# Z-Zheng/ever

Measured on AMD Instinct MI355X. Metric: 512x512 tiles/sec fwd+bwd, FarSeg-R50, higher is better.
Workload: dtype f32; 1 GPU; FarSeg ResNet-50 FPN (FarSegHead defaults, BCE+dice), 3-band 512x512, batch 16/GPU, fwd+bwd+SGD step, inputs resident in HBM; global_batch=16, parallelism=single

## Files before the change

ever_amd/csrc/bn.hip:

```cpp
#include "bn_common.hpp"

namespace evk {

__global__ __launch_bounds__(256) void bn_stats_partial_kernel(const float* __restrict__ x, float* __restrict__ partial,
                                                               int64_t rows, int C, int64_t rows_per_blk, int tpc,
                                                               int rl) {
  __shared__ f32x4 red[2][256];
  const int c4 = C >> 2;
  const int tc = threadIdx.x % tpc, tr = threadIdx.x / tpc;
  const int64_t r0 = (int64_t)blockIdx.x * rows_per_blk;
  const int64_t r1 = min(rows, r0 + rows_per_blk);
  for (int cb = tc; cb < c4; cb += tpc) {
    f32x4 s = {0.f, 0.f, 0.f, 0.f}, q = {0.f, 0.f, 0.f, 0.f};
    const f32x4 pv = *reinterpret_cast<const f32x4*>(x + cb * 4);
    if (tr < rl) {
      int64_t r = r0 + tr;
      const int64_t st = rl;
      for (; r + 3 * st < r1; r += 4 * st) {
        const f32x4 v0 = *reinterpret_cast<const f32x4*>(x + r * C + cb * 4) - pv;
        const f32x4 v1 = *reinterpret_cast<const f32x4*>(x + (r + st) * C + cb * 4) - pv;
        const f32x4 v2 = *reinterpret_cast<const f32x4*>(x + (r + 2 * st) * C + cb * 4) - pv;
        const f32x4 v3 = *reinterpret_cast<const f32x4*>(x + (r + 3 * st) * C + cb * 4) - pv;
        s += (v0 + v1) + (v2 + v3);
        q += (v0 * v0 + v1 * v1) + (v2 * v2 + v3 * v3);
// ... 159 lines not shown
        const f32x4 x0 = bp_ld(x + o0), x1 = bp_ld(x + o1);
        const f32x4 x2 = bp_ld(x + o2), x3 = bp_ld(x + o3);
        f32x4 y0 = zero4, y1 = zero4, y2 = zero4, y3 = zero4;
        if (relu == 1) {
          y0 = bp_ld(y + o0);
          y1 = bp_ld(y + o1);
          y2 = bp_ld(y + o2);
          y3 = bp_ld(y + o3);
        }
        one(g0, x0, y0, o0);
        one(g1, x1, y1, o1);
        one(g2, x2, y2, o2);
        one(g3, x3, y3, o3);
      }
      for (; r < r1; r += st) {
        const size_t o0 = (size_t)r * C + cb * 4;
        const f32x4 g0 = bp_ld(dy + o0);
        const f32x4 x0 = bp_ld(x + o0);
        const f32x4 y0 = (relu == 1) ? bp_ld(y + o0) : zero4;
        one(g0, x0, y0, o0);
      }
    }
    fold_store_record(red, s, q, partial, bn_blk(), C, cb, tc, tr, tpc, rl);
    if constexpr (PK) {
      red[0][threadIdx.x] = gm;
      red[1][threadIdx.x] = xm;
      __syncthreads();
      if (tr == 0) {
        for (int k = 1; k < rl; ++k) {
          const f32x4 a = red[0][k * tpc + tc], b = red[1][k * tpc + tc];
          gm.x = fmaxf(gm.x, a.x); gm.y = fmaxf(gm.y, a.y); gm.z = fmaxf(gm.z, a.z); gm.w = fmaxf(gm.w, a.w);
          xm.x = fmaxf(xm.x, b.x); xm.y = fmaxf(xm.y, b.y); xm.z = fmaxf(xm.z, b.z); xm.w = fmaxf(xm.w, b.w);
        }
        float* o = pmax + (size_t)bn_blk() * 2 * C;
        *reinterpret_cast<f32x4*>(o + cb * 4) = gm;
        *reinterpret_cast<f32x4*>(o + C + cb * 4) = xm;
      }
      __syncthreads();
    }
  }
}

template <int FC = kFinCh>
__global__ __launch_bounds__(256) void bn_bwd_final_kernel(const float* __restrict__ partial, int nblk, int C,
                                                           double inv_rows, const float* __restrict__ gamma,
                                                           const float* __restrict__ invstd,
                                                           float* __restrict__ dgamma, float* __restrict__ dbeta,
                                                           float* __restrict__ coef, int train,
                                                           uint32_t* __restrict__ amax,
                                                           const float* __restrict__ pmax) {
  if (!pmax) zero_amax(amax);
  float gmax = 0.f, xmax = 0.f;
  if (pmax) {
    __shared__ float mred[4][FC];
    const int tc = threadIdx.x % FC, tl = threadIdx.x / FC;
    const int cc = bn_fin_group() * FC + tc;
    if (cc < C) {
      const float* pm = pmax + cc;
      const size_t st = (size_t)2 * C;
      int b = tl;
      for (; b + 3 * (256 / FC) < nblk; b += 4 * (256 / FC)) {
        const float g0 = pm[b * st], g1 = pm[(b + (256 / FC)) * st], g2 = pm[(b + 2 * (256 / FC)) * st],
                    g3 = pm[(b + 3 * (256 / FC)) * st];
        const float x0 = pm[b * st + C], x1 = pm[(b + (256 / FC)) * st + C], x2 = pm[(b + 2 * (256 / FC)) * st + C],
                    x3 = pm[(b + 3 * (256 / FC)) * st + C];
        gmax = fmaxf(gmax, fmaxf(fmaxf(g0, g1), fmaxf(g2, g3)));
        xmax = fmaxf(xmax, fmaxf(fmaxf(x0, x1), fmaxf(x2, x3)));
      }
      for (; b < nblk; b += (256 / FC)) {
        gmax = fmaxf(gmax, pm[b * st]);
        xmax = fmaxf(xmax, pm[b * st + C]);
      }
    }
    auto mx = [](float a, float b) { return fmaxf(a, b); };
    gmax = fold_channel_lanes<FC>(gmax, mred, mx);
    xmax = fold_channel_lanes<FC>(xmax, mred, mx);
  }
  int c;
  double s, q;
  if (!reduce_partials<FC>(partial, nblk, C, c, s, q)) return;
  if (dbeta) dbeta[c] = (float)s;
  if (dgamma) dgamma[c] = (float)q;
  const float g = gamma ? gamma[c] : 1.f;
  const float k0 = g * invstd[c], k1 = train ? (float)(s * inv_rows) : 0.f, k2 = train ? (float)(q * inv_rows) : 0.f;
  coef[c] = k0;
  coef[C + c] = k1;
  coef[2 * C + c] = k2;
  if (pmax) {
    const float bound = fabsf(k0) * (gmax + fabsf(k1) + xmax * fabsf(k2));
    uint32_t bits = __builtin_bit_cast(uint32_t, bound);
    if (bound != bound) bits = 0x7fc00000u;
    if (bits) atomicMax(&amax[0], bits);
  }
}

template <bool PK>
__global__ __launch_bounds__(256) void bn_bwd_apply_kernel(const float* __restrict__ dy, const float* __restrict__ x,
                                                           const float* __restrict__ y, const float* __restrict__ mean,
                                                           const float* __restrict__ invstd,
                                                           const float* __restrict__ coef,
                                                           const float* __restrict__ gamma,
                                                           const float* __restrict__ beta, float* __restrict__ dx,
                                                           size_t n4, int C, int relu, uint32_t* __restrict__ amax,
                                                           const uint32_t* __restrict__ bits = nullptr) {
  const size_t base = (size_t)bn_blk() * 256;
  const size_t i = base + threadIdx.x;
  const bool valid = i < n4;
  f32x4 out = {0.f, 0.f, 0.f, 0.f};
  float pk_inv = 1.f;
  if constexpr (PK) pk_inv = op_scale(amax[0]).inv;
  if (valid) {
    const int c4 = C >> 2;
    const int c = chunk_of(base, c4);
// ... 94 lines not shown
  const double unbias = rows > 1.0 ? rows / (rows - 1.0) : 1.0;
  if (running_mean) running_mean[c] = (1.f - momentum) * running_mean[c] + momentum * meanf;
  if (running_var) running_var[c] = (1.f - momentum) * running_var[c] + momentum * (float)(var * unbias);
  const float g = gamma ? gamma[c] : 1.f, bb = beta ? beta[c] : 0.f;
  const float sc = g * invstd;
  scale_shift[c] = sc;
  scale_shift[C + c] = bb - meanf * sc;
  if (pack) {
    const float bound = fabsf(sc) * (E * 1.001f + fabsf((float)(piv - mean))) + fabsf(bb);
    uint32_t bits = __builtin_bit_cast(uint32_t, bound);
    if (bound != bound) bits = 0x7fc00000u;
    if (bits) atomicMax(&amax[0], bits);
  }
}


static int parts_final_lanes(int nparts) { return nparts >= 1024 ? 256 : (nparts >= 512 ? 128 : 32); }

void launch_parts_final(hipStream_t st, const float* parts, int nparts, int C, double rows, const float* gamma,
                        const float* beta, float* running_mean, float* running_var, float momentum, float eps,
                        float* save_mean, float* save_invstd, float* scale_shift, uint32_t* amax, int pack) {
  const int fl = parts_final_lanes(nparts);
#define EVK_PARTS_FINAL(FC, FL)                                                                                            \
  hipLaunchKernelGGL((bn_parts_final_kernel<FC, FL>), dim3((C + FC - 1) / FC), dim3(256), 0, st, parts, nparts, C, rows, gamma, \
                     beta, running_mean, running_var, momentum, eps, save_mean, save_invstd, scale_shift, amax, pack)
  if (fl == 256) EVK_PARTS_FINAL(1, 256);
  else if (fl == 128) EVK_PARTS_FINAL(2, 128);
  else EVK_PARTS_FINAL(8, 32);
#undef EVK_PARTS_FINAL
}

void launch_bn_bwd_final(hipStream_t st, const float* partial, int nblk, int C, int64_t rows, const float* gamma,
                         const float* invstd, float* dgamma, float* dbeta, float* coef, int train, uint32_t* amax,
                         const float* pmax) {
  hipLaunchKernelGGL(bn_bwd_final_kernel<kFinCh>, dim3((C + kFinCh - 1) / kFinCh), dim3(256), 0, st, partial, nblk, C,
                     1.0 / (double)rows, gamma, invstd, dgamma, dbeta, coef, train ? 1 : 0, amax, pmax);
}

static void launch_bn_apply(hipStream_t st, bool pack, const float* x, const float* residual, const float* scale_shift,
                            float* y, int64_t rows, int C, uint32_t flags, uint32_t* amax, uint32_t* relu_bits = nullptr) {
  const size_t n4 = (size_t)rows * C / 4;
  EVK_BN_LAUNCH_PK(bn_apply_kernel, pack, dim3(oneshot_grid(n4)), 0, st, x, residual, scale_shift, y, n4, C,
                   (flags & EVK_BN_RELU) ? 1 : 0, amax, relu_bits);
}

}

using namespace evk;

extern "C" size_t evk_bn_workspace_bytes(int64_t rows, int32_t C) {
  return rows > 0 && C > 0 ? BnWorkspace::bytes(C) : 0;
}

extern "C" int evk_bn_plan(int64_t rows, int32_t C, int32_t kind, int32_t* out) {
  EVK_REQUIRE(out, EVK_E_INVALID, "bn_plan: null pointer");
  int rc = bn_check("bn_plan", rows, C, nullptr, 0, 0);
  if (rc) return rc;
  EVK_REQUIRE(kind >= 0 && kind <= 2 && (kind == 0 || rows < 0x7fffffffLL), EVK_E_UNSUPPORTED,
              "bn_plan: rows=%lld C=%d kind=%d", (long long)rows, C, kind);
  if (kind == 2) {
    const int fl = parts_final_lanes((int)rows), fc = 256 / fl;
    out[0] = (C + fc - 1) / fc;
    out[2] = fc;
    out[3] = fl;
    out[1] = out[4] = out[5] = 0;
    return EVK_OK;
  }
  const BnPlan pl = kind ? bn_plan(rows, C, 65536, kMaxStatBlocks) : bn_plan(rows, C);
  EVK_REQUIRE(pl.rows_per_blk <= 0x7fffffffLL, EVK_E_UNSUPPORTED, "bn_plan: rows=%lld do not fit the answer", (long long)rows);
  out[0] = pl.nblk;
  out[1] = (int32_t)pl.rows_per_blk;
  out[2] = pl.tpc;
  out[3] = pl.rl;
  out[4] = out[5] = 0;
  if (kind == 1 && rows % 4 == 0) {
    int nblk, qpb;
    bn_quad_split(rows, pl, nblk, qpb);
    out[4] = nblk;
    out[5] = qpb;
  }
  return EVK_OK;
}

extern "C" int evk_bn_fwd_train(const float* x, const float* residual, const float* gamma, const float* beta,
                                float* running_mean, float* running_var, float momentum, float eps, float* y,
                                float* save_mean, float* save_invstd, int64_t rows, int32_t C, uint32_t flags,
                                void* workspace, size_t workspace_bytes, uint32_t* y_absmax, void* stream) {
  EVK_REQUIRE(x && y && save_mean && save_invstd, EVK_E_INVALID, "bn_fwd_train: null pointer");
  int rc = bn_check("bn_fwd_train", rows, C, workspace, workspace_bytes, BnWorkspace::bytes(C));
  if (rc) return rc;
  hipStream_t st = (hipStream_t)stream;
  const BnPlan pl = bn_plan(rows, C);
  const BnWorkspace ws(workspace, C);
  hipLaunchKernelGGL(bn_stats_partial_kernel, dim3(pl.nblk), dim3(256), 0, st, x, ws.partial, rows, C, pl.rows_per_blk,
                     pl.tpc, pl.rl);
  rc = check_launch("bn_stats_partial");
  if (rc) return rc;
  const double unbias = rows > 1 ? (double)rows / (double)(rows - 1) : 1.0;
  hipLaunchKernelGGL(bn_stats_final_kernel, dim3((C + kFinCh - 1) / kFinCh), dim3(256), 0, st, x, ws.partial, pl.nblk, C,
                     1.0 / (double)rows, unbias, gamma, beta, running_mean, running_var, momentum, eps, save_mean,
                     save_invstd, ws.coef, y_absmax);
  rc = check_launch("bn_stats_final");
  if (rc) return rc;
  launch_bn_apply(st, false, x, residual, ws.coef, y, rows, C, flags, y_absmax);
  return check_launch("bn_apply");
}

extern "C" int evk_bn_fwd_train_parts_bits(const float* x, const float* residual, const float* gamma, const float* beta,
                                           float* running_mean, float* running_var, float momentum, float eps, float* y,
                                           float* save_mean, float* save_invstd, int64_t rows, int32_t C, uint32_t flags,
                                           const float* parts, int32_t nparts, void* workspace, size_t workspace_bytes,
                                           uint32_t* y_absmax, uint32_t* relu_bits, void* stream) {
  EVK_REQUIRE(x && y && save_mean && save_invstd && parts && nparts > 0, EVK_E_INVALID, "bn_fwd_train_parts: bad argument");
  int rc = bn_check("bn_fwd_train_parts", rows, C, workspace, workspace_bytes, BnWorkspace::bytes(C));
  if (rc) return rc;
  const bool pack = (flags & EVK_BN_PACK_Y) != 0;
  EVK_REQUIRE(!pack || (y_absmax && !residual), EVK_E_INVALID,
              "bn_fwd_train_parts: EVK_BN_PACK_Y needs y_absmax (slots zero on entry) and no residual");
  hipStream_t st = (hipStream_t)stream;
  float* scale_shift = BnWorkspace(workspace, C).coef;
  launch_parts_final(st, parts, nparts, C, (double)rows, gamma, beta, running_mean, running_var, momentum, eps, save_mean,
                     save_invstd, scale_shift, y_absmax, pack ? 1 : 0);
  rc = check_launch("bn_parts_final");
  if (rc) return rc;
  launch_bn_apply(st, pack, x, residual, scale_shift, y, rows, C, flags, y_absmax, relu_bits);
  return check_launch("bn_apply");
}
extern "C" int evk_bn_fwd_train_parts(const float* x, const float* residual, const float* gamma, const float* beta,
                                      float* running_mean, float* running_var, float momentum, float eps, float* y,
                                      float* save_mean, float* save_invstd, int64_t rows, int32_t C, uint32_t flags,
                                      const float* parts, int32_t nparts, void* workspace, size_t workspace_bytes,
                                      uint32_t* y_absmax, void* stream) {
// ... 10 lines not shown
  int rc = bn_check("bn_fwd_eval", rows, C, workspace, workspace_bytes, 2 * (size_t)C * sizeof(float));
  if (rc) return rc;
  hipStream_t st = (hipStream_t)stream;
  float* scale_shift = (float*)workspace;
  hipLaunchKernelGGL(bn_eval_coef_kernel, dim3((C + 255) / 256), dim3(256), 0, st, gamma, beta, running_mean,
                     running_var, eps, C, scale_shift, save_mean, save_invstd, y_absmax);
  rc = check_launch("bn_eval_coef");
  if (rc) return rc;
  launch_bn_apply(st, false, x, residual, scale_shift, y, rows, C, flags, y_absmax);
  return check_launch("bn_apply");
}

extern "C" int evk_bn_bwd_bits(const float* dy, const float* x, const float* y, const float* gamma, const float* beta,
                               const float* save_mean, const float* save_invstd, float* dx, float* d_residual,
                               float* dgamma, float* dbeta, int64_t rows, int32_t C, uint32_t flags, int32_t train,
                               void* workspace, size_t workspace_bytes, uint32_t* dx_absmax, const uint32_t* relu_bits,
                               void* stream) {
  EVK_REQUIRE(dy && x && save_mean && save_invstd && dx, EVK_E_INVALID, "bn_bwd: null pointer");
  const int relu = relu_bits ? 3 : ((flags & EVK_BN_RELU) ? (y ? 1 : 2) : 0);
  EVK_REQUIRE(relu != 2 || !d_residual, EVK_E_INVALID,
              "bn_bwd: a residual branch needs the forward output y (or its ReLU bits) for the mask");
  int rc = bn_check("bn_bwd", rows, C, workspace, workspace_bytes, BnWorkspace::bytes(C));
  if (rc) return rc;
  hipStream_t st = (hipStream_t)stream;
  const BnPlan pl = bn_plan(rows, C);
  const BnWorkspace ws(workspace, C);
  const bool pack = (flags & EVK_BN_PACK_DX) != 0;
  EVK_REQUIRE(!pack || dx_absmax, EVK_E_INVALID, "bn_bwd: EVK_BN_PACK_DX needs dx_absmax (slots zero on entry)");
  float* pmax = pack ? ws.pmax : nullptr;
  EVK_BN_LAUNCH_PK(bn_bwd_partial_kernel, pack, dim3(pl.nblk), 0, st, dy, x, y, save_mean, save_invstd, gamma, beta, d_residual,
                   ws.partial, rows, C, pl.rows_per_blk, pl.tpc, pl.rl, relu, pmax, relu_bits);
  rc = check_launch("bn_bwd_partial");
  if (rc) return rc;
  launch_bn_bwd_final(st, ws.partial, pl.nblk, C, rows, gamma, save_invstd, dgamma, dbeta, ws.coef, train, dx_absmax, pmax);
  rc = check_launch("bn_bwd_final");
  if (rc) return rc;
  const size_t n4 = (size_t)rows * C / 4;
  const float* gsrc = d_residual ? d_residual : dy;
  const int relu3 = d_residual ? 0 : relu;
  EVK_BN_LAUNCH_PK(bn_bwd_apply_kernel, pack, dim3(oneshot_grid(n4)), 0, st, gsrc, x, y, save_mean, save_invstd, ws.coef, gamma,
                   beta, dx, n4, C, relu3, dx_absmax, relu_bits);
  return check_launch("bn_bwd_apply");
}

extern "C" int evk_bn_bwd(const float* dy, const float* x, const float* y, const float* gamma, const float* beta,
                          const float* save_mean, const float* save_invstd, float* dx, float* d_residual,
                          float* dgamma, float* dbeta, int64_t rows, int32_t C, uint32_t flags, int32_t train,
                          void* workspace, size_t workspace_bytes, uint32_t* dx_absmax, void* stream) {
  return evk_bn_bwd_bits(dy, x, y, gamma, beta, save_mean, save_invstd, dx, d_residual, dgamma, dbeta, rows, C, flags, train,
                         workspace, workspace_bytes, dx_absmax, nullptr, stream);
}

extern "C" int evk_bn_finalize_parts(const float* parts, int32_t nparts, int32_t C, int64_t rows, const float* gamma,
                                     const float* beta, float* running_mean, float* running_var, float momentum, float eps,
                                     float* save_mean, float* save_invstd, float* scale_shift, void* stream) {
  EVK_REQUIRE(parts && nparts > 0 && save_mean && save_invstd && scale_shift, EVK_E_INVALID, "bn_finalize_parts: null pointer");
  int rc = bn_check("bn_finalize_parts", rows, C, nullptr, 0, 0);
  if (rc) return rc;
  launch_parts_final((hipStream_t)stream, parts, nparts, C, (double)rows, gamma, beta, running_mean, running_var, momentum, eps,
                     save_mean, save_invstd, scale_shift, nullptr, 0);
  return check_launch("bn_parts_final");
}
extern "C" int evk_bn_bwd_from_partials(const float* g, const float* x, const float* gamma, const float* save_mean,
                                        const float* save_invstd, const float* partial, const float* maxima, int32_t nparts,
                                        float* dx, float* dgamma, float* dbeta, int64_t rows, int32_t C, uint32_t flags,
                                        int32_t train, void* workspace, size_t workspace_bytes, uint32_t* dx_absmax,
                                        void* stream) {
  EVK_REQUIRE(g && x && save_mean && save_invstd && partial && dx && nparts > 0, EVK_E_INVALID, "bn_bwd_from_partials: null pointer");
  int rc = bn_check("bn_bwd_from_partials", rows, C, workspace, workspace_bytes, (size_t)16 * C * sizeof(float));
  if (rc) return rc;
  const bool pack = (flags & EVK_BN_PACK_DX) != 0;
  EVK_REQUIRE(!pack || (dx_absmax && maxima), EVK_E_INVALID,
              "bn_bwd_from_partials: EVK_BN_PACK_DX needs dx_absmax (slots zero on entry) and the maxima");
  hipStream_t st = (hipStream_t)stream;
  float* coef = (float*)workspace;
  launch_bn_bwd_final(st, partial, nparts, C, rows, gamma, save_invstd, dgamma, dbeta, coef, train, dx_absmax,
                      pack ? maxima : nullptr);
  rc = check_launch("bn_bwd_final");
  if (rc) return rc;
  const size_t n4 = (size_t)rows * C / 4;
  EVK_BN_LAUNCH_PK(bn_bwd_apply_kernel, pack, dim3(oneshot_grid(n4)), 0, st, g, x, (const float*)nullptr, save_mean, save_invstd,
                   coef, gamma, (const float*)nullptr, dx, n4, C, 0, dx_absmax, (const uint32_t*)nullptr);
  return check_launch("bn_bwd_apply");
}

namespace evk {
__global__ __launch_bounds__(256) void relu_bits_apply_kernel(const float* __restrict__ g, const uint32_t* __restrict__ bits,
                                                              float* __restrict__ out, size_t n4) {
  const size_t i = (size_t)blockIdx.x * 256 + threadIdx.x;
  if (i < n4) reinterpret_cast<f32x4*>(out)[i] = relu_bits_mask(reinterpret_cast<const f32x4*>(g)[i], bits, i);
}
}
extern "C" size_t evk_relu_bits_bytes(int64_t n) { return n > 0 ? relu_bits_words(((size_t)n + 3) / 4) * sizeof(uint32_t) : 0; }
extern "C" int evk_relu_bits_apply(const float* g, const uint32_t* bits, float* out, int64_t n, void* stream) {
  EVK_REQUIRE(g && bits && out && n > 0 && n % 4 == 0, EVK_E_INVALID, "relu_bits_apply: null pointer or n %% 4 != 0");
  const size_t n4 = (size_t)n / 4;
  hipLaunchKernelGGL(relu_bits_apply_kernel, dim3(oneshot_grid(n4)), dim3(256), 0, (hipStream_t)stream, g, bits, out, n4);
  return check_launch("relu_bits_apply");
}

namespace evk {

__global__ __launch_bounds__(256) void bn_local_final_kernel(const float* __restrict__ x, const float* __restrict__ partial,
                                                             int nblk, int C, double rows, double* __restrict__ stats) {
  int c;
  double s, q;
  if (!reduce_partials(partial, nblk, C, c, s, q)) return;
  const double dm = s / rows;
  stats[c] = (double)x[c] + dm;
  double m2 = q - s * dm;
// ... 10 lines not shown
}
__global__ __launch_bounds__(256) void bn_bwd_sums_final_kernel(const float* __restrict__ partial, int nblk, int C,
                                                                double* __restrict__ sums) {
  int c;
  double s, q;
  if (!reduce_partials(partial, nblk, C, c, s, q)) return;
  sums[c] = s;
  sums[C + c] = q;
}
__global__ void bn_bwd_coef_kernel(const float* __restrict__ gamma, const float* __restrict__ invstd,
                                   const float* __restrict__ mean_g, const float* __restrict__ mean_gx, int C,
                                   float* __restrict__ coef) {
  const int c = blockIdx.x * blockDim.x + threadIdx.x;
  if (c >= C) return;
  coef[c] = (gamma ? gamma[c] : 1.f) * invstd[c];
  coef[C + c] = mean_g[c];
  coef[2 * C + c] = mean_gx[c];
}

}

extern "C" int evk_bn_local_stats(const float* x, double* stats, int64_t rows, int32_t C, void* workspace,
                                  size_t workspace_bytes, void* stream) {
  EVK_REQUIRE(x && stats, EVK_E_INVALID, "bn_local_stats: null pointer");
  int rc = bn_check("bn_local_stats", rows, C, workspace, workspace_bytes, BnWorkspace::bytes(C));
  if (rc) return rc;
  hipStream_t st = (hipStream_t)stream;
  const BnPlan pl = bn_plan(rows, C);
  float* partial = (float*)workspace;
  hipLaunchKernelGGL(bn_stats_partial_kernel, dim3(pl.nblk), dim3(256), 0, st, x, partial, rows, C, pl.rows_per_blk,
                     pl.tpc, pl.rl);
  rc = check_launch("bn_stats_partial");
  if (rc) return rc;
  hipLaunchKernelGGL(bn_local_final_kernel, dim3((C + kFinCh - 1) / kFinCh), dim3(256), 0, st, x, (const float*)partial,
                     pl.nblk, C, (double)rows, stats);
  return check_launch("bn_local_stats");
}

extern "C" int evk_bn_apply_stats(const float* x, const float* residual, const float* gamma, const float* beta,
                                  const float* mean, const float* invstd, float* y, int64_t rows, int32_t C,
                                  uint32_t flags, void* workspace, size_t workspace_bytes, void* stream) {
  EVK_REQUIRE(x && y && mean && invstd, EVK_E_INVALID, "bn_apply_stats: null pointer");
  int rc = bn_check("bn_apply_stats", rows, C, workspace, workspace_bytes, BnWorkspace::bytes(C));
  if (rc) return rc;
  hipStream_t st = (hipStream_t)stream;
  float* scale_shift = (float*)workspace;
  hipLaunchKernelGGL(bn_coef_from_stats_kernel, dim3((C + 255) / 256), dim3(256), 0, st, gamma, beta, mean, invstd, C,
                     scale_shift);
  rc = check_launch("bn_coef_from_stats");
  if (rc) return rc;
  launch_bn_apply(st, false, x, residual, scale_shift, y, rows, C, flags, nullptr);
  return check_launch("bn_apply_stats");
}

extern "C" int evk_bn_bwd_local_sums(const float* dy, const float* x, const float* y, const float* gamma,
                                     const float* beta, const float* mean, const float* invstd, float* d_residual,
                                     double* sums, int64_t rows, int32_t C, uint32_t flags, void* workspace,
                                     size_t workspace_bytes, void* stream) {
  EVK_REQUIRE(dy && x && mean && invstd && sums, EVK_E_INVALID, "bn_bwd_local_sums: null pointer");
  const int relu = (flags & EVK_BN_RELU) ? (y ? 1 : 2) : 0;
  EVK_REQUIRE(relu != 2 || !d_residual, EVK_E_INVALID, "bn_bwd_local_sums: a residual branch needs y for the ReLU mask");
  int rc = bn_check("bn_bwd_local_sums", rows, C, workspace, workspace_bytes, BnWorkspace::bytes(C));
  if (rc) return rc;
  hipStream_t st = (hipStream_t)stream;
  const BnPlan pl = bn_plan(rows, C);
  float* partial = (float*)workspace;
  hipLaunchKernelGGL(bn_bwd_partial_kernel<false>, dim3(pl.nblk), dim3(256), 0, st, dy, x, y, mean, invstd, gamma, beta,
                     d_residual, partial, rows, C, pl.rows_per_blk, pl.tpc, pl.rl, relu, (float*)nullptr);
  rc = check_launch("bn_bwd_partial");
  if (rc) return rc;
  hipLaunchKernelGGL(bn_bwd_sums_final_kernel, dim3((C + kFinCh - 1) / kFinCh), dim3(256), 0, st, (const float*)partial,
                     pl.nblk, C, sums);
  return check_launch("bn_bwd_local_sums");
}

extern "C" int evk_bn_bwd_apply_sums(const float* dy, const float* x, const float* y, const float* gamma,
                                     const float* beta, const float* mean, const float* invstd, const float* mean_g,
                                     const float* mean_gx, float* dx, int64_t rows, int32_t C, uint32_t flags,
                                     void* workspace, size_t workspace_bytes, void* stream) {
  EVK_REQUIRE(dy && x && mean && invstd && mean_g && mean_gx && dx, EVK_E_INVALID, "bn_bwd_apply_sums: null pointer");
  const int relu = (flags & EVK_BN_RELU) ? (y ? 1 : 2) : 0;
  int rc = bn_check("bn_bwd_apply_sums", rows, C, workspace, workspace_bytes, BnWorkspace::bytes(C));
  if (rc) return rc;
  hipStream_t st = (hipStream_t)stream;
  float* coef = (float*)workspace;
  hipLaunchKernelGGL(bn_bwd_coef_kernel, dim3((C + 255) / 256), dim3(256), 0, st, gamma, invstd, mean_g, mean_gx, C, coef);
  rc = check_launch("bn_bwd_coef");
  if (rc) return rc;
  const size_t n4 = (size_t)rows * C / 4;
  hipLaunchKernelGGL(bn_bwd_apply_kernel<false>, dim3(oneshot_grid(n4)), dim3(256), 0, st, dy, x, y, mean,
                     invstd, (const float*)coef, gamma, beta, dx, n4, C, relu, (uint32_t*)nullptr);
  return check_launch("bn_bwd_apply_sums");
}
```

ever_amd/csrc/bn_common.hpp:

```cpp
#pragma once
#include "x3_common.hpp"

namespace evk {

__device__ __forceinline__ unsigned bn_blk() { return gridDim.x - 1u - blockIdx.x; }

__device__ __forceinline__ int bn_fin_group() { return xcd_remap((int)blockIdx.x, (int)gridDim.x); }

__device__ __forceinline__ f32x4 bn_ld(const float* p, size_t i) {
  return __builtin_nontemporal_load(reinterpret_cast<const f32x4*>(p) + i);
}

constexpr int kMaxStatBlocks = 2048;

__device__ __forceinline__ void zero_amax(uint32_t* __restrict__ amax) {
  if (amax && blockIdx.x == 0 && threadIdx.x < kAmaxSlots) amax[threadIdx.x * kAmaxStride] = 0;
}

struct BnPlan {
  int nblk;
  int64_t rows_per_blk;
  int tpc, rl;
};
inline BnPlan bn_plan(int64_t rows, int C, int64_t per_override = 0, int64_t cap_override = 0) {
  BnPlan p;
  const int c4 = C / 4;
  p.tpc = c4 < 256 ? c4 : 256;
  p.rl = 256 / p.tpc;
  constexpr int64_t per = 32768;
  const int64_t per_e = per_override > 0 ? per_override : per;
  int64_t nb = (rows * (int64_t)C + per_e - 1) / per_e;
  constexpr int64_t cap = 512;
  if (nb > (cap_override > 0 ? cap_override : cap)) nb = cap_override > 0 ? cap_override : cap;
  if (nb > kMaxStatBlocks) nb = kMaxStatBlocks;
  if (nb < 1) nb = 1;
  int64_t rpb = (rows + nb - 1) / nb;
  rpb = ((rpb + p.rl - 1) / p.rl) * p.rl;
  p.rows_per_blk = rpb;
  p.nblk = (int)((rows + rpb - 1) / rpb);
  return p;
}

inline void bn_quad_split(int64_t rows, const BnPlan& pl, int& nblk, int& qpb) {
  const int quads = (int)(rows / 4);
  qpb = (quads + pl.nblk - 1) / pl.nblk;
  qpb = ((qpb + pl.rl - 1) / pl.rl) * pl.rl;
  nblk = (quads + qpb - 1) / qpb;
}

inline unsigned oneshot_grid(size_t n4) { return (unsigned)((n4 + 255) / 256); }

struct BnWorkspace {
  float *partial, *coef, *pmax;
  static size_t bytes(int C) { return ((size_t)kMaxStatBlocks * 4 * C + 8 * (size_t)C) * sizeof(float); }
  BnWorkspace(void* ws, int C)
      : partial((float*)ws), coef(partial + (size_t)kMaxStatBlocks * 2 * C), pmax(coef + 8 * (size_t)C) {}
};

inline int bn_check(const char* what, int64_t rows, int32_t C, const void* ws, size_t ws_bytes, size_t need) {
  EVK_REQUIRE(rows > 0 && C > 0 && C % 4 == 0 && C <= 2048, EVK_E_UNSUPPORTED, "%s: rows=%lld C=%d", what, (long long)rows,
              C);
  EVK_REQUIRE(!need || (ws && ws_bytes >= need), EVK_E_WORKSPACE, "%s: workspace too small", what);
  return EVK_OK;
}

#define EVK_BN_LAUNCH_PK(kernel, pack, grid, lds, st, ...)                                   \
  do {                                                                                       \
    if (pack) hipLaunchKernelGGL((kernel<true>), grid, dim3(256), lds, st, __VA_ARGS__);     \
    else hipLaunchKernelGGL((kernel<false>), grid, dim3(256), lds, st, __VA_ARGS__);         \
  } while (0)

__device__ __forceinline__ f32x4 relu_mask(f32x4 g, const f32x4 yy) {
  g.x = yy.x > 0.f ? g.x : 0.f; g.y = yy.y > 0.f ? g.y : 0.f;
  g.z = yy.z > 0.f ? g.z : 0.f; g.w = yy.w > 0.f ? g.w : 0.f;
  return g;
}

__device__ __forceinline__ void fold_store_record(f32x4 (*red)[256], f32x4 s, f32x4 q, float* rec, size_t blk, int C, int cb,
                                                  int tc, int tr, int tpc, int rl) {
  red[0][threadIdx.x] = s;
  red[1][threadIdx.x] = q;
  __syncthreads();
  if (tr == 0) {
    for (int k = 1; k < rl; ++k) {
      s += red[0][k * tpc + tc];
      q += red[1][k * tpc + tc];
    }
    float* o = rec + blk * 2 * C;
    *reinterpret_cast<f32x4*>(o + cb * 4) = s;
    *reinterpret_cast<f32x4*>(o + C + cb * 4) = q;
  }
  __syncthreads();
}

constexpr int kFinCh = 8;
template <int FC, typename T, typename Op>
__device__ __forceinline__ T fold_channel_lanes(T v, T (*lds)[FC], Op op) {
#pragma unroll
  for (int o = FC; o < 64; o <<= 1) v = op(v, __shfl_xor(v, o, 64));
  const int lane = threadIdx.x & 63, w = threadIdx.x >> 6;
  if (lane < FC) lds[w][lane] = v;
  __syncthreads();
  const int tc = threadIdx.x % FC;
  const T r = op(op(lds[0][tc], lds[1][tc]), op(lds[2][tc], lds[3][tc]));
  __syncthreads();
  return r;
}
template <int FC = kFinCh>
__device__ __forceinline__ bool reduce_partials(const float* __restrict__ partial, int nblk, int C, int& c, double& s,
                                                double& q) {
  __shared__ double red[4][FC];
  const int tc = threadIdx.x % FC, tl = threadIdx.x / FC;
  c = bn_fin_group() * FC + tc;
  s = 0.0;
  q = 0.0;
  if (c < C) {
    const float* ps = partial + c;
    const size_t st = (size_t)2 * C;
    int b = tl;
    for (; b + 3 * (256 / FC) < nblk; b += 4 * (256 / FC)) {
      const float s0 = ps[b * st], s1 = ps[(b + (256 / FC)) * st], s2 = ps[(b + 2 * (256 / FC)) * st],
                  s3 = ps[(b + 3 * (256 / FC)) * st];
      const float q0 = ps[b * st + C], q1 = ps[(b + (256 / FC)) * st + C], q2 = ps[(b + 2 * (256 / FC)) * st + C],
                  q3 = ps[(b + 3 * (256 / FC)) * st + C];
      s += ((double)s0 + (double)s1) + ((double)s2 + (double)s3);
      q += ((double)q0 + (double)q1) + ((double)q2 + (double)q3);
    }
    for (; b < nblk; b += (256 / FC)) {
      s += (double)ps[b * st];
      q += (double)ps[b * st + C];
    }
  }
  auto add = [](double a, double b) { return a + b; };
  s = fold_channel_lanes<FC>(s, red, add);
  q = fold_channel_lanes<FC>(q, red, add);
  return tl == 0 && c < C;
}

__device__ __forceinline__ void block_absmax(const f32x4 v, bool valid, uint32_t* __restrict__ amax) {
  __shared__ uint32_t red[4];
  uint32_t m = 0;
  if (valid) {
    m = __builtin_bit_cast(uint32_t, fmaxf(fmaxf(fabsf(v.x), fabsf(v.y)), fmaxf(fabsf(v.z), fabsf(v.w))));
    if (v.x != v.x || v.y != v.y || v.z != v.z || v.w != v.w) m = 0x7fc00000u;
  }
#pragma unroll
  for (int o = 32; o > 0; o >>= 1) m = max(m, (uint32_t)__shfl_xor((int)m, o, 64));
  if ((threadIdx.x & 63) == 0) red[threadIdx.x >> 6] = m;
  __syncthreads();
  if (threadIdx.x == 0) {
    const uint32_t t = max(max(red[0], red[1]), max(red[2], red[3]));
    if (t) atomicMax(&amax[(blockIdx.x & (kAmaxSlots - 1)) * kAmaxStride], t);
  }
}

void launch_parts_final(hipStream_t st, const float* parts, int nparts, int C, double rows, const float* gamma,
                        const float* beta, float* running_mean, float* running_var, float momentum, float eps,
                        float* save_mean, float* save_invstd, float* scale_shift, uint32_t* amax, int pack);
void launch_bn_bwd_final(hipStream_t st, const float* partial, int nblk, int C, int64_t rows, const float* gamma,
                         const float* invstd, float* dgamma, float* dbeta, float* coef, int train, uint32_t* amax,
                         const float* pmax);

}
```

ever_amd/csrc/bn_dot.hip:

```cpp
#include "bn_common.hpp"

namespace evk {
constexpr int kDotMaxK = 16;
__device__ __forceinline__ float wave_sum_f(float v) {
#pragma unroll
  for (int o = 32; o > 0; o >>= 1) v += __shfl_xor(v, o, 64);
  return v;
}
__device__ __forceinline__ f32x4 bn_relu_4(const f32x4 z, const f32x4 sc, const f32x4 sh) {
  f32x4 y = z * sc + sh;
  y.x = fmaxf(y.x, 0.f); y.y = fmaxf(y.y, 0.f); y.z = fmaxf(y.z, 0.f); y.w = fmaxf(y.w, 0.f);
  return y;
}
template <int NCH, int KT>
__global__ __launch_bounds__(256) void bn_relu_dot_fwd_kernel(const float* __restrict__ z, const float* __restrict__ ss,
                                                              const float* __restrict__ w, const float* __restrict__ bias,
                                                              float* __restrict__ out, size_t npix, int C, int K,
                                                              size_t pix_per_blk) {
  const int c4 = C >> 2, lane = threadIdx.x & 63, wave = threadIdx.x >> 6;
  const f32x4 zero4 = {0.f, 0.f, 0.f, 0.f};
  f32x4 sc[NCH], sh[NCH], wk[NCH][KT];
#pragma unroll
  for (int j = 0; j < NCH; ++j) {
    const int cb = lane + 64 * j;
// ... 105 lines not shown
  for (size_t pix = p0 + wave; pix < p1; pix += 8) {
    f32x4 za[NCH], zb[NCH];
    float da[KT], dbb[KT];
    fetch(pix, za, da);
    fetch(pix + 4, zb, dbb);
    one(za, da);
    one(zb, dbb);
  }
  float* my = sdot + (size_t)wave * R * C;
#pragma unroll
  for (int j = 0; j < NCH; ++j) {
    const int cb = lane + 64 * j;
    if (cb < c4) {
      *reinterpret_cast<f32x4*>(my + cb * 4) = sg[j];
      *reinterpret_cast<f32x4*>(my + C + cb * 4) = sq[j];
      *reinterpret_cast<f32x4*>(my + 2 * C + cb * 4) = mg[j];
      *reinterpret_cast<f32x4*>(my + 3 * C + cb * 4) = mx[j];
#pragma unroll
      for (int k = 0; k < KT; ++k)
        if (k < K) *reinterpret_cast<f32x4*>(my + (size_t)(4 + k) * C + cb * 4) = dwa[j][k];
    }
  }
  __shared__ float sdb[4][kDotMaxK];
  if (lane == 0)
#pragma unroll
    for (int k = 0; k < KT; ++k) sdb[wave][k] = db[k];
  __syncthreads();
  const size_t W = (size_t)R * C, blk = blockIdx.x;
  for (int c = threadIdx.x; c < C; c += 256) {
    auto fold = [&](int k) { return (sdot[(size_t)k * C + c] + sdot[W + (size_t)k * C + c]) + (sdot[2 * W + (size_t)k * C + c] + sdot[3 * W + (size_t)k * C + c]); };
    auto fmx = [&](int k) {
      return fmaxf(fmaxf(sdot[(size_t)k * C + c], sdot[W + (size_t)k * C + c]), fmaxf(sdot[2 * W + (size_t)k * C + c], sdot[3 * W + (size_t)k * C + c]));
    };
    bnp[blk * 2 * C + c] = fold(0);
    bnp[blk * 2 * C + C + c] = fold(1);
    bnm[blk * 2 * C + c] = fmx(2);
    bnm[blk * 2 * C + C + c] = fmx(3);
    for (int k = 0; k < K; ++k) dwp[(blk * K + k) * C + c] = fold(4 + k);
  }
  if (threadIdx.x < K) dbp[blk * K + threadIdx.x] = (sdb[0][threadIdx.x] + sdb[1][threadIdx.x]) + (sdb[2][threadIdx.x] + sdb[3][threadIdx.x]);
}
__global__ __launch_bounds__(256) void bn_relu_dot_bwd_wfinal_kernel(const float* __restrict__ dwp, const float* __restrict__ dbp,
                                                                     float* __restrict__ dw, float* __restrict__ dbias, int nblk,
                                                                     int C, int K) {
  __shared__ double red[32][8];
  const int to = threadIdx.x & 7, tl = threadIdx.x >> 3;
  const int i = blockIdx.x * 8 + to;
  const int nw = K * C;
  double s = 0.0;
  if (i < nw) {
    for (int b = tl; b < nblk; b += 32) s += (double)dwp[(size_t)b * nw + i];
  } else if (i < nw + K) {
    for (int b = tl; b < nblk; b += 32) s += (double)dbp[(size_t)b * K + (i - nw)];
  }
  red[tl][to] = s;
  __syncthreads();
  if (tl == 0) {
    for (int k = 1; k < 32; ++k) s += red[k][to];
    if (i < nw) dw[i] = (float)s;
    else if (i < nw + K && dbias) dbias[i - nw] = (float)s;
  }
}
template <bool PK>
__global__ __launch_bounds__(256) void bn_relu_dot_bwd_apply_kernel(const float* __restrict__ dl, const float* __restrict__ z,
                                                                    const float* __restrict__ ss, const float* __restrict__ mean,
                                                                    const float* __restrict__ invstd,
                                                                    const float* __restrict__ coef, const float* __restrict__ w,
                                                                    float* __restrict__ dz, size_t n4, int C, int K,
                                                                    uint32_t* __restrict__ amax) {
  const size_t i = (size_t)blockIdx.x * 256 + threadIdx.x;
// ... 67 lines not shown
  const size_t nb = (size_t)dot_blocks((size_t)rows);
  return (nb * (size_t)(4 + K) * C + nb * K + (size_t)16 * C) * sizeof(float);
}
extern "C" int evk_bn_relu_dot_bwd(const float* dl, const float* z, const float* scale_shift, const float* gamma,
                                   const float* save_mean, const float* save_invstd, const float* w, float* dz, float* dgamma,
                                   float* dbeta, float* dw, float* dbias, int64_t rows, int32_t C, int32_t K, uint32_t flags,
                                   void* workspace, size_t workspace_bytes, uint32_t* dx_absmax, void* stream) {
  EVK_REQUIRE(dl && z && scale_shift && save_mean && save_invstd && w && dz && dw, EVK_E_INVALID, "bn_relu_dot_bwd: null pointer");
  EVK_REQUIRE(rows > 0 && C > 0 && C % 4 == 0 && C <= 1024 && K > 0 && K <= kDotMaxK, EVK_E_UNSUPPORTED,
              "bn_relu_dot_bwd: C=%d K=%d", C, K);
  EVK_REQUIRE(workspace && workspace_bytes >= evk_bn_relu_dot_workspace_bytes(rows, C, K), EVK_E_WORKSPACE,
              "bn_relu_dot_bwd: workspace too small");
  const bool pack = (flags & EVK_BN_PACK_DX) != 0;
  EVK_REQUIRE(!pack || dx_absmax, EVK_E_INVALID, "bn_relu_dot_bwd: EVK_BN_PACK_DX needs dx_absmax (slots zero on entry)");
  hipStream_t st = (hipStream_t)stream;
  const int nb = dot_blocks((size_t)rows);
  const size_t ppb = ((size_t)rows + nb - 1) / nb;
  float* bnp = (float*)workspace;
  float* bnm = bnp + (size_t)nb * 2 * C;
  float* dwp = bnm + (size_t)nb * 2 * C;
  float* dbp = dwp + (size_t)nb * K * C;
  float* coef = dbp + (size_t)nb * K;
  const size_t lds = (size_t)4 * (4 + K) * C * sizeof(float);
  EVK_REQUIRE(lds <= 64 * 1024, EVK_E_UNSUPPORTED, "bn_relu_dot_bwd: C=%d K=%d do not fit the LDS", C, K);
  int nch, kt;
  EVK_REQUIRE(dot_variant(C, K, nch, kt), EVK_E_UNSUPPORTED, "bn_relu_dot_bwd: C=%d K=%d has no instantiation", C, K);
#define EVK_DOT_PARTIAL(NCH, KT)                                                                                          \
  hipLaunchKernelGGL((bn_relu_dot_bwd_partial_kernel<NCH, KT>), dim3(nb), dim3(256), lds, st, dl, z, scale_shift, save_mean, \
                     save_invstd, w, bnp, bnm, dwp, dbp, (size_t)rows, C, K, ppb)
  EVK_DOT_DISPATCH(nch, kt, EVK_DOT_PARTIAL);
#undef EVK_DOT_PARTIAL
  int rc = check_launch("bn_relu_dot_bwd_partial");
  if (rc) return rc;
  launch_bn_bwd_final(st, bnp, nb, C, rows, gamma, save_invstd, dgamma, dbeta, coef, 1, dx_absmax, pack ? bnm : nullptr);
  rc = check_launch("bn_bwd_final");
  if (rc) return rc;
  hipLaunchKernelGGL(bn_relu_dot_bwd_wfinal_kernel, dim3((K * C + K + 7) / 8), dim3(256), 0, st, (const float*)dwp,
                     (const float*)dbp, dw, dbias, nb, C, K);
  rc = check_launch("bn_relu_dot_bwd_wfinal");
  if (rc) return rc;
  const size_t n4 = (size_t)rows * C / 4;
  EVK_BN_LAUNCH_PK(bn_relu_dot_bwd_apply_kernel, pack, dim3(oneshot_grid(n4)), 0, st, dl, z, scale_shift, save_mean, save_invstd,
                   (const float*)coef, w, dz, n4, C, K, dx_absmax);
  return check_launch("bn_relu_dot_bwd_apply");
}
```

ever_amd/csrc/bn_pool.hip:

```cpp
#include "bn_common.hpp"

namespace evk {

template <int BIT>
__device__ __forceinline__ f32x4 pool_ld(const float* p) {
  if constexpr ((5 & BIT) != 0) return __builtin_nontemporal_load(reinterpret_cast<const f32x4*>(p));
  return *reinterpret_cast<const f32x4*>(p);
}

__global__ __launch_bounds__(256) void bn_relu_pool_fwd_kernel(const float* __restrict__ x,
                                                               const float* __restrict__ scale_shift,
                                                               float* __restrict__ y, uint8_t* __restrict__ code, int N,
                                                               int H, int W, int C, int Ho, int Wo,
                                                               uint32_t* __restrict__ amax) {
  const int c4 = C >> 2;
  const uint32_t total = (uint32_t)N * Ho * Wo * c4;
  const uint32_t i = blockIdx.x * 256u + threadIdx.x;
  const bool valid = i < total;
  f32x4 best = {0.f, 0.f, 0.f, 0.f};
  if (valid) {
    const int cb = (int)(i % (uint32_t)c4);
    uint32_t pix = i / (uint32_t)c4;
    const int ox = (int)(pix % (uint32_t)Wo);
    pix /= (uint32_t)Wo;
// ... 272 lines not shown
  const int Ho = (H - 1) / 2 + 1, Wo = (W - 1) / 2 + 1;
  const size_t total = (size_t)N * Ho * Wo * (C / 4);
  hipLaunchKernelGGL(bn_relu_pool_fwd_kernel, dim3(oneshot_grid(total)), dim3(256), 0, st, x, scale_shift, y, code, N, H, W, C,
                     Ho, Wo, y_absmax);
  return check_launch("bn_relu_pool_fwd");
}

extern "C" int evk_bn_relu_pool_bwd(const float* dp, const uint8_t* code, const float* x, const float* gamma,
                                    const float* beta, const float* save_mean, const float* save_invstd, float* dx,
                                    float* dgamma, float* dbeta, int32_t N, int32_t H, int32_t W, int32_t C, int32_t train,
                                    void* workspace, size_t workspace_bytes, uint32_t* dx_absmax, void* stream) {
  EVK_REQUIRE(dp && code && x && save_mean && save_invstd && dx, EVK_E_INVALID, "bn_relu_pool_bwd: null pointer");
  const int64_t rows = (int64_t)N * H * W;
  EVK_REQUIRE(N > 0 && H > 0 && W > 0 && C > 0 && rows * (C / 4) < 0x7fffffffLL, EVK_E_UNSUPPORTED,
              "bn_relu_pool_bwd: N=%d H=%d W=%d C=%d", N, H, W, C);
  int rc = bn_check("bn_relu_pool_bwd", rows, C, workspace, workspace_bytes, BnWorkspace::bytes(C));
  if (rc) return rc;
  hipStream_t st = (hipStream_t)stream;
  const BnPlan pl = bn_plan(rows, C, 65536, kMaxStatBlocks);
  const BnWorkspace ws(workspace, C);
  const int Ho = (H - 1) / 2 + 1, Wo = (W - 1) / 2 + 1;
  const bool quad = (H % 2 == 0) && (W % 2 == 0);
  const int quads = (int)(rows / 4);
  int nblk = pl.nblk, qpb = 0;
  if (quad) bn_quad_split(rows, pl, nblk, qpb);
  if (quad)
    hipLaunchKernelGGL(bn_pool_bwd_partial_quad_kernel, dim3(nblk), dim3(256), 0, st, dp, code, x, save_mean, save_invstd,
                       gamma, beta, ws.partial, quads, H, W, C, Ho, Wo, qpb, pl.tpc, pl.rl);
  else
    hipLaunchKernelGGL(bn_pool_bwd_partial_kernel, dim3(pl.nblk), dim3(256), 0, st, dp, code, x, save_mean, save_invstd, gamma,
                       beta, ws.partial, (int)rows, H, W, C, Ho, Wo, (int)pl.rows_per_blk, pl.tpc, pl.rl);
  rc = check_launch("bn_pool_bwd_partial");
  if (rc) return rc;
  launch_bn_bwd_final(st, ws.partial, nblk, C, rows, gamma, save_invstd, dgamma, dbeta, ws.coef, train, dx_absmax, nullptr);
  rc = check_launch("bn_bwd_final");
  if (rc) return rc;
  const uint32_t n4 = (uint32_t)(rows * (C / 4));
  if (quad)
    hipLaunchKernelGGL(bn_pool_bwd_apply_quad_kernel, dim3(oneshot_grid(n4 / 4)), dim3(256), 0, st, dp, code, x, save_mean,
                       save_invstd, (const float*)ws.coef, gamma, beta, dx, n4 / 4, H, W, C, Ho, Wo, dx_absmax);
  else
    hipLaunchKernelGGL(bn_pool_bwd_apply_kernel, dim3(oneshot_grid(n4)), dim3(256), 0, st, dp, code, x, save_mean, save_invstd,
                       (const float*)ws.coef, gamma, beta, dx, n4, H, W, C, Ho, Wo, dx_absmax);
  return check_launch("bn_pool_bwd_apply");
}
```

Baseline: 562.2 tiles/s.

## Store BN partial records channel-group-major and fold them with vectorized group reduction

Partial sum/sumsq and max records written by the BN partial kernels now use a layout indexed by channel group of four, then block, then stat. This makes each group's records contiguous across blocks. The final kernels read these records as f32x4 with unrolled loads and reduce them through shared memory and cross-lane shuffles, replacing strided per-channel scalar reads. The goal is better-coalesced, fewer memory transactions in the small final-reduction kernels. Callers that receive externally supplied partials (the parts path) keep the old row-major reducer. This risks a mismatch if any producer still writes the old layout.

```diff
diff --git a/ever_amd/csrc/bn.hip b/ever_amd/csrc/bn.hip
--- a/ever_amd/csrc/bn.hip
+++ b/ever_amd/csrc/bn.hip
@@ -215,16 +215,16 @@
           gm.x = fmaxf(gm.x, a.x); gm.y = fmaxf(gm.y, a.y); gm.z = fmaxf(gm.z, a.z); gm.w = fmaxf(gm.w, a.w);
           xm.x = fmaxf(xm.x, b.x); xm.y = fmaxf(xm.y, b.y); xm.z = fmaxf(xm.z, b.z); xm.w = fmaxf(xm.w, b.w);
         }
-        float* o = pmax + (size_t)bn_blk() * 2 * C;
-        *reinterpret_cast<f32x4*>(o + cb * 4) = gm;
-        *reinterpret_cast<f32x4*>(o + C + cb * 4) = xm;
+        float* o = pmax + bn_rec_index(cb * 4, bn_blk(), 0, gridDim.x);
+        *reinterpret_cast<f32x4*>(o) = gm;
+        *reinterpret_cast<f32x4*>(o + 4) = xm;
       }
       __syncthreads();
     }
   }
 }
 
-template <int FC = kFinCh>
+template <int F, bool GR>
 __global__ __launch_bounds__(256) void bn_bwd_final_kernel(const float* __restrict__ partial, int nblk, int C,
                                                            double inv_rows, const float* __restrict__ gamma,
                                                            const float* __restrict__ invstd,
@@ -234,34 +234,41 @@
                                                            const float* __restrict__ pmax) {
   if (!pmax) zero_amax(amax);
   float gmax = 0.f, xmax = 0.f;
-  if (pmax) {
-    __shared__ float mred[4][FC];
-    const int tc = threadIdx.x % FC, tl = threadIdx.x / FC;
-    const int cc = bn_fin_group() * FC + tc;
-    if (cc < C) {
-      const float* pm = pmax + cc;
-      const size_t st = (size_t)2 * C;
-      int b = tl;
-      for (; b + 3 * (256 / FC) < nblk; b += 4 * (256 / FC)) {
-        const float g0 = pm[b * st], g1 = pm[(b + (256 / FC)) * st], g2 = pm[(b + 2 * (256 / FC)) * st],
-                    g3 = pm[(b + 3 * (256 / FC)) * st];
-        const float x0 = pm[b * st + C], x1 = pm[(b + (256 / FC)) * st + C], x2 = pm[(b + 2 * (256 / FC)) * st + C],
-                    x3 = pm[(b + 3 * (256 / FC)) * st + C];
-        gmax = fmaxf(gmax, fmaxf(fmaxf(g0, g1), fmaxf(g2, g3)));
-        xmax = fmaxf(xmax, fmaxf(fmaxf(x0, x1), fmaxf(x2, x3)));
-      }
-      for (; b < nblk; b += (256 / FC)) {
-        gmax = fmaxf(gmax, pm[b * st]);
-        xmax = fmaxf(xmax, pm[b * st + C]);
-      }
-    }
-    auto mx = [](float a, float b) { return fmaxf(a, b); };
-    gmax = fold_channel_lanes<FC>(gmax, mred, mx);
-    xmax = fold_channel_lanes<FC>(xmax, mred, mx);
-  }
   int c;
   double s, q;
-  if (!reduce_partials<FC>(partial, nblk, C, c, s, q)) return;
+  bool own;
+  if constexpr (GR) {
+    if (pmax) fold_group_records<F>(pmax, nblk, C, c, gmax, xmax, 0.f, [](float a, float b) { return fmaxf(a, b); });
+    own = fold_group_records<F>(partial, nblk, C, c, s, q, 0.0, [](double a, double b) { return a + b; });
+  } else {
+    if (pmax) {
+      __shared__ float mred[4][F];
+      const int tc = threadIdx.x % F, tl = threadIdx.x / F;
+      const int cc = bn_fin_group() * F + tc;
+      if (cc < C) {
+        const float* pm = pmax + cc;
+        const size_t st = (size_t)2 * C;
+        int b = tl;
+        for (; b + 3 * (256 / F) < nblk; b += 4 * (256 / F)) {
+          const float g0 = pm[b * st], g1 = pm[(b + (256 / F)) * st], g2 = pm[(b + 2 * (256 / F)) * st],
+                      g3 = pm[(b + 3 * (256 / F)) * st];
+          const float x0 = pm[b * st + C], x1 = pm[(b + (256 / F)) * st + C], x2 = pm[(b + 2 * (256 / F)) * st + C],
+                      x3 = pm[(b + 3 * (256 / F)) * st + C];
+          gmax = fmaxf(gmax, fmaxf(fmaxf(g0, g1), fmaxf(g2, g3)));
+          xmax = fmaxf(xmax, fmaxf(fmaxf(x0, x1), fmaxf(x2, x3)));
+        }
+        for (; b < nblk; b += (256 / F)) {
+          gmax = fmaxf(gmax, pm[b * st]);
+          xmax = fmaxf(xmax, pm[b * st + C]);
+        }
+      }
+      auto mx = [](float a, float b) { return fmaxf(a, b); };
+      gmax = fold_channel_lanes<F>(gmax, mred, mx);
+      xmax = fold_channel_lanes<F>(xmax, mred, mx);
+    }
+    own = reduce_partials_rows<F>(partial, nblk, C, c, s, q);
+  }
+  if (!own) return;
   if (dbeta) dbeta[c] = (float)s;
   if (dgamma) dgamma[c] = (float)q;
   const float g = gamma ? gamma[c] : 1.f;
@@ -422,9 +429,13 @@
 
 void launch_bn_bwd_final(hipStream_t st, const float* partial, int nblk, int C, int64_t rows, const float* gamma,
                          const float* invstd, float* dgamma, float* dbeta, float* coef, int train, uint32_t* amax,
-                         const float* pmax) {
-  hipLaunchKernelGGL(bn_bwd_final_kernel<kFinCh>, dim3((C + kFinCh - 1) / kFinCh), dim3(256), 0, st, partial, nblk, C,
-                     1.0 / (double)rows, gamma, invstd, dgamma, dbeta, coef, train ? 1 : 0, amax, pmax);
+                         const float* pmax, bool grouped) {
+  if (grouped)
+    hipLaunchKernelGGL((bn_bwd_final_kernel<kFinGr, true>), dim3(bn_fin_grid(C)), dim3(256), 0, st, partial, nblk, C,
+                       1.0 / (double)rows, gamma, invstd, dgamma, dbeta, coef, train ? 1 : 0, amax, pmax);
+  else
+    hipLaunchKernelGGL((bn_bwd_final_kernel<kFinCh, false>), dim3((C + kFinCh - 1) / kFinCh), dim3(256), 0, st, partial, nblk, C,
+                       1.0 / (double)rows, gamma, invstd, dgamma, dbeta, coef, train ? 1 : 0, amax, pmax);
 }
 
 static void launch_bn_apply(hipStream_t st, bool pack, const float* x, const float* residual, const float* scale_shift,
@@ -487,7 +498,7 @@
   rc = check_launch("bn_stats_partial");
   if (rc) return rc;
   const double unbias = rows > 1 ? (double)rows / (double)(rows - 1) : 1.0;
-  hipLaunchKernelGGL(bn_stats_final_kernel, dim3((C + kFinCh - 1) / kFinCh), dim3(256), 0, st, x, ws.partial, pl.nblk, C,
+  hipLaunchKernelGGL(bn_stats_final_kernel, dim3(bn_fin_grid(C)), dim3(256), 0, st, x, ws.partial, pl.nblk, C,
                      1.0 / (double)rows, unbias, gamma, beta, running_mean, running_var, momentum, eps, save_mean,
                      save_invstd, ws.coef, y_absmax);
   rc = check_launch("bn_stats_final");
@@ -564,7 +575,7 @@
                    ws.partial, rows, C, pl.rows_per_blk, pl.tpc, pl.rl, relu, pmax, relu_bits);
   rc = check_launch("bn_bwd_partial");
   if (rc) return rc;
-  launch_bn_bwd_final(st, ws.partial, pl.nblk, C, rows, gamma, save_invstd, dgamma, dbeta, ws.coef, train, dx_absmax, pmax);
+  launch_bn_bwd_final(st, ws.partial, pl.nblk, C, rows, gamma, save_invstd, dgamma, dbeta, ws.coef, train, dx_absmax, pmax, true);
   rc = check_launch("bn_bwd_final");
   if (rc) return rc;
   const size_t n4 = (size_t)rows * C / 4;
@@ -607,7 +618,7 @@
   hipStream_t st = (hipStream_t)stream;
   float* coef = (float*)workspace;
   launch_bn_bwd_final(st, partial, nparts, C, rows, gamma, save_invstd, dgamma, dbeta, coef, train, dx_absmax,
-                      pack ? maxima : nullptr);
+                      pack ? maxima : nullptr, false);
   rc = check_launch("bn_bwd_final");
   if (rc) return rc;
   const size_t n4 = (size_t)rows * C / 4;
@@ -684,7 +695,7 @@
                      pl.tpc, pl.rl);
   rc = check_launch("bn_stats_partial");
   if (rc) return rc;
-  hipLaunchKernelGGL(bn_local_final_kernel, dim3((C + kFinCh - 1) / kFinCh), dim3(256), 0, st, x, (const float*)partial,
+  hipLaunchKernelGGL(bn_local_final_kernel, dim3(bn_fin_grid(C)), dim3(256), 0, st, x, (const float*)partial,
                      pl.nblk, C, (double)rows, stats);
   return check_launch("bn_local_stats");
 }
@@ -721,7 +732,7 @@
                      d_residual, partial, rows, C, pl.rows_per_blk, pl.tpc, pl.rl, relu, (float*)nullptr);
   rc = check_launch("bn_bwd_partial");
   if (rc) return rc;
-  hipLaunchKernelGGL(bn_bwd_sums_final_kernel, dim3((C + kFinCh - 1) / kFinCh), dim3(256), 0, st, (const float*)partial,
+  hipLaunchKernelGGL(bn_bwd_sums_final_kernel, dim3(bn_fin_grid(C)), dim3(256), 0, st, (const float*)partial,
                      pl.nblk, C, sums);
   return check_launch("bn_bwd_local_sums");
 }
diff --git a/ever_amd/csrc/bn_common.hpp b/ever_amd/csrc/bn_common.hpp
--- a/ever_amd/csrc/bn_common.hpp
+++ b/ever_amd/csrc/bn_common.hpp
@@ -50,6 +50,10 @@
 
 inline unsigned oneshot_grid(size_t n4) { return (unsigned)((n4 + 255) / 256); }
 
+__host__ __device__ __forceinline__ size_t bn_rec_index(int c, size_t blk, int stat, size_t nblk) {
+  return (((size_t)(c >> 2) * nblk + blk) * 2 + stat) * 4 + (c & 3);
+}
+
 struct BnWorkspace {
   float *partial, *coef, *pmax;
   static size_t bytes(int C) { return ((size_t)kMaxStatBlocks * 4 * C + 8 * (size_t)C) * sizeof(float); }
@@ -86,9 +90,9 @@
       s += red[0][k * tpc + tc];
       q += red[1][k * tpc + tc];
     }
-    float* o = rec + blk * 2 * C;
-    *reinterpret_cast<f32x4*>(o + cb * 4) = s;
-    *reinterpret_cast<f32x4*>(o + C + cb * 4) = q;
+    float* o = rec + bn_rec_index(cb * 4, blk, 0, gridDim.x);
+    *reinterpret_cast<f32x4*>(o) = s;
+    *reinterpret_cast<f32x4*>(o + 4) = q;
   }
   __syncthreads();
 }
@@ -107,7 +111,7 @@
   return r;
 }
 template <int FC = kFinCh>
-__device__ __forceinline__ bool reduce_partials(const float* __restrict__ partial, int nblk, int C, int& c, double& s,
+__device__ __forceinline__ bool reduce_partials_rows(const float* __restrict__ partial, int nblk, int C, int& c, double& s,
                                                 double& q) {
   __shared__ double red[4][FC];
   const int tc = threadIdx.x % FC, tl = threadIdx.x / FC;
@@ -137,6 +141,56 @@
   return tl == 0 && c < C;
 }
 
+
+constexpr int kFinGr = 4;
+inline unsigned bn_fin_grid(int C) { return (unsigned)((C / 4 + kFinGr - 1) / kFinGr); }
+template <int FG = kFinGr, typename T, typename Op>
+__device__ __forceinline__ bool fold_group_records(const float* __restrict__ rec, int nblk, int C, int& c, T& a, T& b, T zero,
+                                                   Op op) {
+  constexpr int TG = 256 / FG, TPC = 32 / FG;
+  static_assert(FG >= 1 && FG <= 32 && (FG & (FG - 1)) == 0, "32 / FG threads per (channel, stat) column");
+  __shared__ T lds[4][256];
+  {
+    const int l = threadIdx.x % TG;
+    const int grp = bn_fin_group() * FG + threadIdx.x / TG;
+    T v[4] = {zero, zero, zero, zero};
+    if (grp < (C >> 2)) {
+      const f32x4* p = reinterpret_cast<const f32x4*>(rec) + (size_t)grp * nblk * 2;
+      const f32x4 none = {(float)zero, (float)zero, (float)zero, (float)zero};
+      const int n = 2 * nblk;
+      for (int i = l; i < n; i += 8 * TG) {
+        f32x4 e[8];
+#pragma unroll
+        for (int j = 0; j < 8; ++j) e[j] = i + j * TG < n ? p[i + j * TG] : none;
+#pragma unroll
+        for (int k = 0; k < 4; ++k)
+          v[k] = op(v[k], op(op(op((T)e[0][k], (T)e[1][k]), op((T)e[2][k], (T)e[3][k])),
+                             op(op((T)e[4][k], (T)e[5][k]), op((T)e[6][k], (T)e[7][k]))));
+      }
+    }
+#pragma unroll
+    for (int k = 0; k < 4; ++k) lds[k][threadIdx.x] = v[k];
+  }
+  __syncthreads();
+  const int ch = threadIdx.x / (2 * TPC), stat = (threadIdx.x / TPC) & 1, part = threadIdx.x % TPC;
+  const int g = ch >> 2;
+  const T* col = &lds[ch & 3][g * TG + 2 * part + stat];
+  T r = op(op(col[0], col[2 * TPC]), op(col[4 * TPC], col[6 * TPC]));
+#pragma unroll
+  for (int o = 1; o < TPC; o <<= 1) r = op(r, __shfl_xor(r, o, 64));
+  const T other = __shfl_xor(r, TPC, 64);
+  a = stat ? other : r;
+  b = stat ? r : other;
+  __syncthreads();
+  const int grp = bn_fin_group() * FG + g;
+  c = grp * 4 + (ch & 3);
+  return threadIdx.x % (2 * TPC) == 0 && grp < (C >> 2);
+}
+__device__ __forceinline__ bool reduce_partials(const float* __restrict__ partial, int nblk, int C, int& c, double& s,
+                                                double& q) {
+  return fold_group_records<kFinGr>(partial, nblk, C, c, s, q, 0.0, [](double x, double y) { return x + y; });
+}
+
 __device__ __forceinline__ void block_absmax(const f32x4 v, bool valid, uint32_t* __restrict__ amax) {
   __shared__ uint32_t red[4];
   uint32_t m = 0;
@@ -159,6 +213,6 @@
                         float* save_mean, float* save_invstd, float* scale_shift, uint32_t* amax, int pack);
 void launch_bn_bwd_final(hipStream_t st, const float* partial, int nblk, int C, int64_t rows, const float* gamma,
                          const float* invstd, float* dgamma, float* dbeta, float* coef, int train, uint32_t* amax,
-                         const float* pmax);
-
-}
+                         const float* pmax, bool grouped);
+
+}
diff --git a/ever_amd/csrc/bn_dot.hip b/ever_amd/csrc/bn_dot.hip
--- a/ever_amd/csrc/bn_dot.hip
+++ b/ever_amd/csrc/bn_dot.hip
@@ -161,10 +161,10 @@
     auto fmx = [&](int k) {
       return fmaxf(fmaxf(sdot[(size_t)k * C + c], sdot[W + (size_t)k * C + c]), fmaxf(sdot[2 * W + (size_t)k * C + c], sdot[3 * W + (size_t)k * C + c]));
     };
-    bnp[blk * 2 * C + c] = fold(0);
-    bnp[blk * 2 * C + C + c] = fold(1);
-    bnm[blk * 2 * C + c] = fmx(2);
-    bnm[blk * 2 * C + C + c] = fmx(3);
+    bnp[bn_rec_index(c, blk, 0, gridDim.x)] = fold(0);
+    bnp[bn_rec_index(c, blk, 1, gridDim.x)] = fold(1);
+    bnm[bn_rec_index(c, blk, 0, gridDim.x)] = fmx(2);
+    bnm[bn_rec_index(c, blk, 1, gridDim.x)] = fmx(3);
     for (int k = 0; k < K; ++k) dwp[(blk * K + k) * C + c] = fold(4 + k);
   }
   if (threadIdx.x < K) dbp[blk * K + threadIdx.x] = (sdb[0][threadIdx.x] + sdb[1][threadIdx.x]) + (sdb[2][threadIdx.x] + sdb[3][threadIdx.x]);
@@ -298,7 +298,7 @@
 #undef EVK_DOT_PARTIAL
   int rc = check_launch("bn_relu_dot_bwd_partial");
   if (rc) return rc;
-  launch_bn_bwd_final(st, bnp, nb, C, rows, gamma, save_invstd, dgamma, dbeta, coef, 1, dx_absmax, pack ? bnm : nullptr);
+  launch_bn_bwd_final(st, bnp, nb, C, rows, gamma, save_invstd, dgamma, dbeta, coef, 1, dx_absmax, pack ? bnm : nullptr, true);
   rc = check_launch("bn_bwd_final");
   if (rc) return rc;
   hipLaunchKernelGGL(bn_relu_dot_bwd_wfinal_kernel, dim3((K * C + K + 7) / 8), dim3(256), 0, st, (const float*)dwp,
diff --git a/ever_amd/csrc/bn_pool.hip b/ever_amd/csrc/bn_pool.hip
--- a/ever_amd/csrc/bn_pool.hip
+++ b/ever_amd/csrc/bn_pool.hip
@@ -328,7 +328,7 @@
                        beta, ws.partial, (int)rows, H, W, C, Ho, Wo, (int)pl.rows_per_blk, pl.tpc, pl.rl);
   rc = check_launch("bn_pool_bwd_partial");
   if (rc) return rc;
-  launch_bn_bwd_final(st, ws.partial, nblk, C, rows, gamma, save_invstd, dgamma, dbeta, ws.coef, train, dx_absmax, nullptr);
+  launch_bn_bwd_final(st, ws.partial, nblk, C, rows, gamma, save_invstd, dgamma, dbeta, ws.coef, train, dx_absmax, nullptr, true);
   rc = check_launch("bn_bwd_final");
   if (rc) return rc;
   const uint32_t n4 = (uint32_t)(rows * (C / 4));
```

Result: no change. 562.0 tiles/s (-0.0%).
